# ZhenlongYuan/DVP-MVS

Measured on AMD Instinct MI355X. Metric: Mpixels/sec/PatchMatch-iteration, higher is better.
Workload: dtype f32

## Files before the change

__graft_entry__.py:

```python
import importlib
import os
import subprocess
import sys

ROOT = os.path.dirname(os.path.abspath(__file__))
if ROOT not in sys.path:
    sys.path.insert(0, ROOT)


def build() -> None:
    subprocess.check_call(["make", "-s", "-C", os.path.join(ROOT, "dvp-mvs_amd", "csrc")])
    host = os.path.join(ROOT, "dvp-mvs_amd", "host")
    if os.path.exists(os.path.join(host, "Makefile")):
        subprocess.check_call(["make", "-s", "-C", host])
    subprocess.check_call(["make", "-s", "-C", os.path.join(ROOT, "oracle")])
    subprocess.check_call(["make", "-s", "-C", os.path.join(ROOT, "tests", "emul")])
    subprocess.check_call(["make", "-s", "-C", os.path.join(ROOT, "tests", "sweep_host")])
    subprocess.check_call(["make", "-s", "-C", os.path.join(ROOT, "tests", "host")])
    subprocess.check_call(["make", "-s", "-C", os.path.join(ROOT, "tests", "half16")])
    subprocess.check_call(["make", "-s", "-C", os.path.join(ROOT, "tests", "jpeg_host")])
    subprocess.check_call(["make", "-s", "-C", os.path.join(ROOT, "tests", "edges_host")])
    subprocess.check_call(["make", "-s", "-C", os.path.join(ROOT, "tests", "viewclean_host")])
    subprocess.check_call(["make", "-s", "-C", os.path.join(ROOT, "tests", "labels_host")])
    subprocess.check_call(["make", "-s", "-C", os.path.join(ROOT, "tests", "pyramid_host")])
    subprocess.check_call(["make", "-s", "-C", os.path.join(ROOT, "tests", "prior_host")])
    subprocess.check_call(["make", "-s", "-C", os.path.join(ROOT, "tests", "reuse_host")])
    subprocess.check_call(["make", "-s", "-C", os.path.join(ROOT, "tests", "devmem_host")])
    subprocess.check_call(["make", "-s", "-C", os.path.join(ROOT, "tests", "jpeg_dec_host")])
    subprocess.check_call(["make", "-s", "-C", os.path.join(ROOT, "tests", "convert_host")])
    subprocess.check_call(["make", "-s", "-C", os.path.join(ROOT, "tests", "undistort_host")])
    pkg = importlib.import_module("dvp-mvs_amd")
    lib = pkg.get_capi().lib()
    missing = [s for s in pkg.get_capi().EXPORTS + pkg.get_capi().EXPORTS_WITH_DIGITS if not hasattr(lib, s)]
    if missing:
        raise RuntimeError("libdvp_mvs_hip.so lacks symbols: %s" % missing)


def smoke() -> None:
    import numpy as np
    pkg = importlib.import_module("dvp-mvs_amd")
    synth, capi = pkg.synth, pkg.get_capi()
    from oracle import oracle as O
    W, H, S = 96, 64, 3
    sc = synth.make_scene(W, H, S)
    p = synth.default_params(S + 1, max_iterations=1, state=synth.FIRST_INIT, use_APD=0)
    p["depth_min"] = np.float32(2.5) * np.float32(0.6)
    p["depth_max"] = np.float32(6.5) * np.float32(1.2)
    state = dict(planes=np.zeros((H * W, 4), np.float32), edge=sc["edge"], label=sc["label"],
                 radius=np.full(H * W, 5, np.int32))
    g = capi.from_scene(sc, p, device=0)
    g.upload_state(**state)
    g.run_patchmatch()
    o = O.from_scene(sc, p)
    o.upload_state(**state)
    o.run_patchmatch()
    pg, po = g.get("planes"), o.get("planes")
    same = (pg.view(np.uint32) == po.view(np.uint32)) | (np.isnan(pg) & np.isnan(po))
    if not same.all():
        raise AssertionError("smoke: HIP planes differ from the oracle in %d values" % int((~same).sum()))
    for n in ("selected_views", "weak_info", "radius"):
        if not (g.get(n) == o.get(n)).all():
            raise AssertionError("smoke: %s differs from the oracle" % n)
    print("smoke ok: %dx%d S=%d bit-exact vs oracle; total %.2f ms" % (W, H, S, g.timings()["total_ms"]))


if __name__ == "__main__":
    build()
    if os.path.exists("/dev/kfd"):
        smoke()
```

dvp-mvs_amd/csrc/dvp_engine.hip:

```cpp
#include "dvp_kernels.hpp"
#include "dvp_ctx.hpp"
#ifdef DVP_PROBE
#include "dvp_probe.inc"
#endif
#include "dvp_pyramid_run.h"
#include <cstring>
#include <thread>
#include <chrono>
#include <algorithm>
#include <cmath>

extern "C" {

int dvp_ctx_create(int device, int width, int height, int num_images, dvp_ctx** out) {
	if (!out) return 1;
	*out = nullptr;
	if (width <= 0 || height <= 0 || num_images < 2 || num_images > DVP_MAX_IMAGES || width > 32767 || height > 32767) {
		g_create_error = "dvp_ctx_create: bad dimensions (2 <= num_images <= 32, sizes <= 32767: short2 pixel coordinates)";
		return 1;
	}
	{
		const unsigned long long pitch = ((unsigned long long)width + 2 * kImgPad + 63) / 64 * 64;
		if (pitch * ((unsigned long long)height + 2 * kImgPad) * 8ull >= (1ull << 32)) {
			g_create_error = "dvp_ctx_create: image too large (a padded row-pair plane must stay below 4 GiB)";
// ... 477 lines not shown
	if (anchor_table_off(c) || c->anchor_tab_valid) return 0;
	const int wc = c->d.weak_black + c->d.weak_red;
	if (grow_anchor_table(c, (size_t)wc)) return 1;
	if (anchor_table_off(c)) return 0;
	c->anchor_tab_valid = true;
	sync_dev_struct(c);
	ListArgs la;
	la.base = 0; la.count = wc; la.iter = 0; la.covered_rows = covered_rows;
	const long long n = (long long)wc * (c->NI - 1) * kAnchors;
	if (n > 0) {
		hipLaunchKernelGGL(dvp_weak_anchor_table, dim3((unsigned)((n + 255) / 256)), dim3(256), 0, c->stream, c->d, la);
		HIP_TRY(c, hipGetLastError());
	}
	return 0;
}

static int grow_weak_phase_buffers(dvp_ctx* c, size_t wc) {
	if (!c->sw.weak_phased || !c->weak_phase_fits || wc <= c->weak_phase_alloc) return 0;
	HIP_TRY(c, hipStreamSynchronize(c->stream));
	dfree(c, &c->weak_rec); dfree(c, &c->weak_ctab); dfree(c, &c->weak_ev);
	c->weak_phase_alloc = 0;
	const size_t cap = std::min<size_t>(c->L, wc + wc / 2), S = (size_t)c->NI - 1;
	if (alloc_group_or_fall_back(c, { areq(&c->weak_rec, cap * sizeof(WeakRec)), areq(&c->weak_ctab, cap * kTaps * kTaps * sizeof(f2)), areq(&c->weak_ev, cap * 8 * S * sizeof(float)) },
			"DVP_TEST_WEAK_PHASE_ALLOC_FAIL", &c->weak_phase_fits, "dvp: no room for the phased weak update's hand-over buffers (%.2f GB); using the one-wave kernel\n", (double)cap * (sizeof(WeakRec) + 288 + 32 * S) / 1e9))
		c->weak_phase_alloc = cap;
	return 0;
}

static void ensure_strong_reuse_buffers(dvp_ctx* c) {
	if (c->reuse_costs || !c->sw.strong_reuse || !c->reuse_fits || strong_form(c->sw, c->NI - 1, c->split_fits, false, 0).kernel != STRONG_SPLIT) return;
	const size_t L = c->L, vec = (size_t)kSlotCount * (c->NI - 1) * L * sizeof(float) + 64 ;
	const size_t Lh = (size_t)((c->W + 1) / 2) * c->H;
	alloc_group_or_fall_back(c, { areq(&c->reuse_costs, vec), areq(&c->reuse_keys, L * kSlotCount * sizeof(PlaneKey)), areq(&c->reuse_hdr, L * sizeof(ReuseHdr), true),
			c->strong_rec ? AllocReq{} : areq(&c->strong_rec, (size_t)SR_FIELDS * Lh * sizeof(*c->strong_rec)) },
		"DVP_TEST_REUSE_ALLOC_FAIL", &c->reuse_fits, "dvp: no room for the strong update's plane cache (%.1f GB); every visit evaluates all its planes\n", (double)(vec + L * (kSlotCount * sizeof(PlaneKey) + sizeof(ReuseHdr))) / 1e9);
}
static void ensure_strong_split_buffers(dvp_ctx* c) {
	if (c->slot_costs || strong_form(c->sw, c->NI - 1, c->split_fits, false, 0).kernel != STRONG_SPLIT) return;
	if (!getenv("DVP_TEST_SPLIT_ALLOC_FAIL")) {
		ensure_strong_reuse_buffers(c);
		if (c->reuse_costs) return;
	}
	const size_t Lh = (size_t)((c->W + 1) / 2) * c->H;
	alloc_group_or_fall_back(c, { areq(&c->slot_costs, (size_t)kSlotCount * (c->NI - 1) * Lh * sizeof(*c->slot_costs) + 64 ),
			areq(&c->strong_rec, (size_t)SR_FIELDS * Lh * sizeof(*c->strong_rec)) },
		"DVP_TEST_SPLIT_ALLOC_FAIL", &c->split_fits, "dvp: no room for the split strong update's cost buffer (%.1f GB); using the monolithic kernel\n", (double)kSlotCount * (c->NI - 1) * Lh * 4 / 1e9);
}
static void ensure_sweep_buffers(dvp_ctx* c) {
	if (c->sweep_cost || !c->sw.sweep_split || !c->sweep_fits) return;
	const size_t L = c->L;
	c->sweep_band_rows = sweep_band_rows(c->sw, c->W, c->H, c->NI - 1);
	const size_t band_px = c->sweep_band_rows > 0 ? (size_t)c->sweep_band_rows * c->W : L;
	alloc_group_or_fall_back(c, { areq(&c->sweep_rec, 2 * L * sizeof(f4)), areq(&c->sweep_pc, 61 * L * sizeof(float)), areq(&c->sweep_cost, sweep_cost_floats(band_px, c->NI - 1) * sizeof(float)) },
		"DVP_TEST_SWEEP_ALLOC_FAIL", &c->sweep_fits, "dvp: no room for the view-compacted DepthToWeak's cost buffer (%.1f GB); using the fused kernel\n", (double)(c->NI - 1) * kSweepFields * L * 4 / 1e9);
}


#define DVP_PICK(NAME, SUF) (c->d.sampler ? NAME##_exact##SUF : NAME##SUF)
#define DVP_PICK_FMT(NAME, TAIL) (fmt == 1 ? DVP_PICK(NAME, _u8##TAIL) : (fmt == 2 ? DVP_PICK(NAME, _f16##TAIL) : DVP_PICK(NAME, TAIL)))

static LaunchArgs make_args(const LaunchGeom& g, int colour, int iter) {
	LaunchArgs a;
	a.tiles_x = g.tiles_x; a.tiles = g.tiles; a.rows = g.rows; a.half = g.half ? 1 : 0;
	a.colour = colour; a.iter = iter;
	return a;
}

static void launch_gen_candidates(dvp_ctx* c, hipStream_t stream, const Dev& d, unsigned blocks, const LaunchArgs& a, const unsigned* list = nullptr, const unsigned* n_list = nullptr) {
	const bool all = gen_candidates_all_views(d);
	const dim3 grid(blocks, all ? (unsigned)((c->NI - 1 + kCandGroup - 1) / kCandGroup) : (unsigned)(c->NI - 1)), block(256);
	if (list) hipLaunchKernelGGL(all ? dvp_gen_candidates_views_list : dvp_gen_candidates_list, grid, block, 0, stream, d, list, n_list);
	else hipLaunchKernelGGL(all ? dvp_gen_candidates_views : dvp_gen_candidates, grid, block, 0, stream, d, a);
}

static int launch_strong_prep(dvp_ctx* c, const LaunchGeom& g, const LaunchArgs& a) {
	EventPair prep;
	prep.stage = DVP_ST_STRONG_PREP;
	HIP_TRY(c, hipEventCreate(&prep.a));
	HIP_TRY(c, hipEventCreate(&prep.b));
	HIP_TRY(c, hipEventRecord(prep.a, c->stream));
	HIP_TRY(c, hipMemcpyAsync(c->planes_snap, c->planes, c->L * 16, hipMemcpyDeviceToDevice, c->stream));
	HIP_TRY(c, hipMemcpyAsync(c->costs_snap, c->costs, c->L * 4, hipMemcpyDeviceToDevice, c->stream));
	ensure_strong_split_buffers(c);
	hipLaunchKernelGGL(dvp_strong_search, dim3(g.grid()), dim3(256), 0, c->stream, c->d, a);
	if (strong_form(c->sw, c->NI - 1, c->split_fits, c->d.reuse_hdr != nullptr, 0).plan) hipLaunchKernelGGL(dvp_strong_plan, dim3(g.grid()), dim3(256), 0, c->stream, c->d, a);
	HIP_TRY(c, hipGetLastError());
	HIP_TRY(c, hipEventRecord(prep.b, c->stream));
	c->events.push_back(prep);
	return 0;
}

static int launch_strong_update(dvp_ctx* c, const LaunchGeom& g, const LaunchArgs& a) {
	const dim3 grid(g.grid()), block(256);
	const dim3 wave_grid((unsigned)((g.grid() + 7) / 8 * 32)), wave_block(64);
	ensure_strong_split_buffers(c);
	const StrongForm f = strong_form(c->sw, c->NI - 1, c->split_fits, c->d.reuse_hdr != nullptr, (unsigned long long)c->pitch * (c->H + 2 * kImgPad) * 8 * c->NI);
	switch (f.kernel) {
	case STRONG_SPLIT:
		if (f.eval_items) hipLaunchKernelGGL(DVP_PICK(dvp_strong_eval_items, ), wave_grid, wave_block, 0, c->stream, c->d, a);
		else hipLaunchKernelGGL(DVP_PICK(dvp_strong_eval, ), wave_grid, wave_block, 0, c->stream, c->d, a);
		hipLaunchKernelGGL(f.decide == 4 ? dvp_strong_decide_v4 : f.decide == 6 ? dvp_strong_decide_v6 : f.decide == 8 ? dvp_strong_decide_v8 : f.decide == 10 ? dvp_strong_decide_v10 :
		                   f.decide == 12 ? dvp_strong_decide_v12 : f.decide == 16 ? dvp_strong_decide_v16 : dvp_strong_decide_wide, grid, block, 0, c->stream, c->d, a);
		if (f.refine_lanes) hipLaunchKernelGGL(DVP_PICK(dvp_strong_refine_lanes, ), wave_grid, wave_block, 0, c->stream, c->d, a);
		else hipLaunchKernelGGL(DVP_PICK(dvp_strong_refine, ), wave_grid, wave_block, 0, c->stream, c->d, a);
		break;
	case STRONG_MONO_V8: hipLaunchKernelGGL(DVP_PICK(dvp_strong_update_v8, ), grid, block, 0, c->stream, c->d, a); break;
	case STRONG_MONO_V16: hipLaunchKernelGGL(DVP_PICK(dvp_strong_update_v16, ), grid, block, 0, c->stream, c->d, a); break;
	case STRONG_MONO: hipLaunchKernelGGL(DVP_PICK(dvp_strong_update, ), grid, block, 0, c->stream, c->d, a); break;
	}
	HIP_TRY(c, hipGetLastError());
	return 0;
}

static int launch_weak_update(dvp_ctx* c, ListArgs la) {
	if (ensure_anchor_table(c, la.covered_rows)) return 1;
	if (c->d.anchor_tab && grow_weak_phase_buffers(c, (size_t)(c->d.weak_black + c->d.weak_red))) return 1;
	const WeakForm f = weak_form(c->sw, c->d.anchor_tab != nullptr, c->weak_phase_fits, la.count);
	const int fmt = dvp_image_format(c);
	const dim3 lg((la.count + 255) / 256), block(256), w64(64), lg64((la.count + 63) / 64);
	switch (f.kernel) {
	case WEAK_PHASED:
#define DVP_GROUP_LAUNCH(NAME, PHASE) { la.group = f.group[PHASE]; la.run = f.run[PHASE]; hipLaunchKernelGGL(DVP_PICK_FMT(NAME, ), dim3((la.count + la.group - 1) / la.group), w64, 0, c->stream, c->d, la); }
		DVP_GROUP_LAUNCH(dvp_weak_eval_candidates, 0)
		hipLaunchKernelGGL(dvp_weak_select_views, lg, block, 0, c->stream, c->d, la);
		DVP_GROUP_LAUNCH(dvp_weak_eval_planes, 1)
		hipLaunchKernelGGL(dvp_weak_make_hypotheses, lg, block, 0, c->stream, c->d, la);
		DVP_GROUP_LAUNCH(dvp_weak_eval_first_view, 2)
		DVP_GROUP_LAUNCH(dvp_weak_eval_survivors, 3)
#undef DVP_GROUP_LAUNCH
		hipLaunchKernelGGL(dvp_weak_adopt, lg, block, 0, c->stream, c->d, la);
		hipLaunchKernelGGL(DVP_PICK(dvp_weak_final_cost, ), lg64, w64, 0, c->stream, c->d, la);
		break;
	case WEAK_WAVE: hipLaunchKernelGGL(DVP_PICK_FMT(dvp_weak_update_wave, ), dim3(la.count), w64, 0, c->stream, c->d, la); break;
	case WEAK_WAVE_NOTAB: hipLaunchKernelGGL(DVP_PICK_FMT(dvp_weak_update_wave, _notab), dim3(la.count), w64, 0, c->stream, c->d, la); break;
	}
	return 0;
}

static int launch_list_site(dvp_ctx* c, int stage, int iter, int colour) {
	const dim3 block(256);
	const size_t words = edge_bits_words(c->W, c->H);
	const dim3 wgrid((unsigned)((words + 255) / 256));
	if (stage == DVP_ST_FIND_NEAREST_STRONG && c->d.weak_black + c->d.weak_red > 0) {
		hipLaunchKernelGGL(dvp_pack_edge_bits, wgrid, block, 0, c->stream, c->weak_info, c->strong_bits, c->W, c->H, edge_tiles_x(c->W), words, (int)DVP_STRONG);
		hipLaunchKernelGGL(dvp_pack_bits_transposed, wgrid, block, 0, c->stream, c->weak_info, c->strong_bits_t, c->W, c->H, edge_tiles_x(c->W), words, (int)DVP_STRONG);
		HIP_TRY(c, hipGetLastError());
	}
	if (stage == DVP_ST_GEN_NEIGHBOURS || stage == DVP_ST_RANSAC_FIT) {
		hipLaunchKernelGGL(dvp_pack_edge_bits, wgrid, block, 0, c->stream, c->edge, c->edge_bits, c->W, c->H, edge_tiles_x(c->W), words, -1);
		HIP_TRY(c, hipGetLastError());
		const int cells = c->d.sat_cells_x * c->d.sat_cells_y;
		hipLaunchKernelGGL(dvp_edge_cell_counts, dim3((cells + 255) / 256), dim3(256), 0, c->stream, c->d);
		hipLaunchKernelGGL(dvp_edge_sat_rows, dim3((c->d.sat_cells_y + 1 + 63) / 64), dim3(64), 0, c->stream, c->d);
		hipLaunchKernelGGL(dvp_edge_sat_cols, dim3((c->d.sat_cells_x + 1 + 63) / 64), dim3(64), 0, c->stream, c->d);
		HIP_TRY(c, hipGetLastError());
		if (stage == DVP_ST_GEN_NEIGHBOURS) {
			hipLaunchKernelGGL(dvp_pack_edge_bits, wgrid, block, 0, c->stream, c->weak_info, c->strong_bits, c->W, c->H, edge_tiles_x(c->W), words, (int)DVP_STRONG);
			HIP_TRY(c, hipGetLastError());
		}
	}
	if (stage == DVP_ST_FIND_NEAREST_STRONG) HIP_TRY(c, hipMemsetAsync(c->weak_nearest_strong, 0xFF, c->L * sizeof(s2), c->stream));
	if (stage == DVP_ST_RANSAC_FIT) HIP_TRY(c, hipMemcpyAsync(c->fit_planes, c->planes, c->L * 16, hipMemcpyDeviceToDevice, c->stream));
	ListArgs la;
	la.iter = iter;
	la.covered_rows = 2 * make_geom(c->W, c->H, true).rows;
	la.base = (stage == DVP_ST_WEAK_UPDATE && colour == 1) ? c->d.weak_black : 0;
	la.count = (stage == DVP_ST_WEAK_UPDATE) ? (colour == 0 ? c->d.weak_black : (colour == 1 ? c->d.weak_red : c->d.weak_black + c->d.weak_red)) : c->d.weak_black + c->d.weak_red;
	if (la.count <= 0) return 0;
// ... 595 lines not shown
```

dvp-mvs_amd/csrc/dvp_kernels.hpp:

```cpp
#ifndef DVP_KERNELS_HPP_
#define DVP_KERNELS_HPP_

#include "dvp_stages.hpp"
#include <hip/hip_runtime.h>

using namespace dvp;

struct LaunchArgs {
	int tiles_x, tiles, rows, half, colour, iter;
};

template <int STAGE, int SMP, int MV = 32>
__device__ __forceinline__ void stage_body(const Dev& d, const LaunchArgs& a) {
	const int lane = threadIdx.x & 63;
	const int wave = threadIdx.x >> 6;
	int px, py;
	unsigned long long n = 0;
	__shared__ f2 lds_tab[stage_uses_tab(STAGE) ? kTaps * kTaps * 256 : 1];
	const PatchTab tab{&lds_tab[stage_uses_tab(STAGE) ? threadIdx.x : 0], 256};
	if (block_to_pixel(blockIdx.x, lane, wave, a.tiles_x, a.tiles, a.rows, a.half, a.colour, d.width, d.height, &px, &py))
		run_pixel<STAGE, SMP, MV>(d, px, py, a.iter, d.eval_counter ? &n : nullptr, tab);
	if (d.eval_counter && n) atomicAdd(d.eval_counter, n);
}

// ... 509 lines not shown
}

extern "C" __global__ void __launch_bounds__(256) dvp_gen_candidates_views(const Dev d, const LaunchArgs a) {
	int px, py;
	if (block_to_pixel(blockIdx.x, threadIdx.x & 63, threadIdx.x >> 6, a.tiles_x, a.tiles, a.rows, 0, 0, d.width, d.height, &px, &py))
		gen_candidates_views_px<kCandGroup>(d, px, py, (int)blockIdx.y * kCandGroup);
}
extern "C" __global__ void __launch_bounds__(256) dvp_gen_candidates_views_list(const Dev d, const unsigned* list, const unsigned* n_list) {
	const unsigned t = blockIdx.x * 256 + threadIdx.x;
	if (t >= *n_list) return;
	const int center = (int)list[t];
	const int py = center / d.width, px = center - py * d.width;
	gen_candidates_views_px<kCandGroup>(d, px, py, (int)blockIdx.y * kCandGroup);
}

extern "C" __global__ void __launch_bounds__(256) dvp_anchor_mask(const Dev d, const ListArgs a, uint8_t* mask) {
	const int t = blockIdx.x * 256 + threadIdx.x;
	if (t >= a.count) return;
	const int center = d.weak_list[a.base + t];
	const s2* nb = d.neighbours + (size_t)d.neighbours_map[center] * DVP_NEIGHBOUR_NUM;
	for (int k = 1; k < DVP_NEIGHBOUR_NUM; ++k) {
		const s2 q = nb[k];
		if (q.x >= 0 && q.y >= 0 && q.x < d.width && q.y < d.height) mask[(size_t)q.y * d.width + q.x] = 1;
	}
}
extern "C" __global__ void __launch_bounds__(256) dvp_mask_compact(const uint8_t* mask, size_t L, unsigned* list, unsigned* n_list) {
	const size_t p = (size_t)blockIdx.x * 256 + threadIdx.x;
	const bool go = p < L && mask[p] != 0;
	const unsigned long long m = __ballot(go);
	if (!m) return;
	const int lane = threadIdx.x & 63;
	unsigned base = 0;
	if (lane == __builtin_ctzll(m)) base = atomicAdd(n_list, (unsigned)__popcll(m));
	base = __shfl(base, __builtin_ctzll(m), 64);
	if (go) list[base + __popcll(m & ((1ull << lane) - 1ull))] = (unsigned)p;
}
extern "C" __global__ void __launch_bounds__(256) dvp_gen_candidates_list(const Dev d, const unsigned* list, const unsigned* n_list) {
	const unsigned t = blockIdx.x * 256 + threadIdx.x;
	if (t >= *n_list) return;
	const int center = (int)list[t];
	const int py = center / d.width, px = center - py * d.width;
	gen_candidates_px(d, px, py, (int)blockIdx.y);
}

extern "C" __global__ void dvp_pack_bits_transposed(const uint8_t* __restrict__ map, uint32_t* __restrict__ bits, int W, int H, int tiles_x, size_t words, int equals) {
	const size_t w = (size_t)blockIdx.x * blockDim.x + threadIdx.x;
	if (w < words) bits[w] = pack_edge_word_t(map, W, H, tiles_x, w, equals);
}

extern "C" __global__ void dvp_edge_cell_counts(const Dev d) {
	const int c = blockIdx.x * blockDim.x + threadIdx.x;
	if (c >= d.sat_cells_x * d.sat_cells_y) return;
	const int cy = c / d.sat_cells_x, cx = c - cy * d.sat_cells_x;
	int n = 0;
	for (int r = 0; r < 8; ++r) {
		const int y = cy * 8 + r;
		if (y >= d.height) break;
		const unsigned w = d.edge_bits[(size_t)(((y >> 5) * d.edge_tiles_x + (cx >> 2)) * 32 + (y & 31))];
		n += __popc((w >> ((cx & 3) * 8)) & 255u);
	}
	d.edge_sat[(cy + 1) * (d.sat_cells_x + 1) + cx + 1] = n;
}
extern "C" __global__ void dvp_edge_sat_rows(const Dev d) {
	const int r = blockIdx.x * blockDim.x + threadIdx.x;
	if (r > d.sat_cells_y) return;
	int* row = d.edge_sat + (size_t)r * (d.sat_cells_x + 1);
	int acc = 0;
	for (int x = 0; x <= d.sat_cells_x; ++x) { acc += (r == 0 || x == 0) ? 0 : row[x]; row[x] = acc; }
}
extern "C" __global__ void dvp_edge_sat_cols(const Dev d) {
	const int x = blockIdx.x * blockDim.x + threadIdx.x;
	if (x > d.sat_cells_x) return;
	const int P = d.sat_cells_x + 1;
	int acc = 0;
	for (int r = 0; r <= d.sat_cells_y; ++r) { acc += d.edge_sat[(size_t)r * P + x]; d.edge_sat[(size_t)r * P + x] = acc; }
}

extern "C" __global__ void __launch_bounds__(256) dvp_strong_search(const Dev d, const LaunchArgs a) {
	int px, py;
	if (block_to_pixel(blockIdx.x, threadIdx.x & 63, threadIdx.x >> 6, a.tiles_x, a.tiles, a.rows, a.half, a.colour, d.width, d.height, &px, &py))
		strong_search_px(d, px, py);
}

extern "C" __global__ void __launch_bounds__(256) dvp_strong_plan(const Dev d, const LaunchArgs a) {
	int px, py;
	if (block_to_pixel(blockIdx.x, threadIdx.x & 63, threadIdx.x >> 6, a.tiles_x, a.tiles, a.rows, a.half, a.colour, d.width, d.height, &px, &py) &&
	    d.weak_info[px + py * d.width] != DVP_WEAK)
		strong_plan_px(d, px, py);
}

extern "C" __global__ void __launch_bounds__(256) dvp_edge_rays(const Dev d, int what) {
	edge_ray_line(d, blockIdx.y, blockIdx.x * blockDim.x + threadIdx.x, what);
}

constexpr int kWeakTile = 16, kWeakSuper = 64, kWeakChunk = 1024;
DVP_HD void weak_slot_origin(int slot, int supers_x, int* tx, int* ty) {
	const int super = slot >> 4, t = slot & 15;
	*tx = (super % supers_x) * kWeakSuper + (t & 3) * kWeakTile;
	*ty = (super / supers_x) * kWeakSuper + (t >> 2) * kWeakTile;
}
extern "C" __global__ void __launch_bounds__(256) dvp_weak_counts(const uint8_t* __restrict__ weak, int W, int H, int supers_x, int n_slots, int n_chunks, int* __restrict__ counts) {
	const int lane = threadIdx.x & 63;
	const int unit = blockIdx.x * 4 + (threadIdx.x >> 6);
	if (unit < n_slots) {
		int tx, ty;
		weak_slot_origin(unit, supers_x, &tx, &ty);
		int nb = 0, nr = 0;
		for (int step = 0; step < 4; ++step) {
			const int x = tx + (lane & 15), y = ty + step * 4 + (lane >> 4);
			const bool wk = x < W && y < H && weak[(size_t)y * W + x] == DVP_WEAK;
			nb += __popcll(__ballot(wk && !((x + y) & 1)));
			nr += __popcll(__ballot(wk && ((x + y) & 1)));
		}
		if (lane == 0) { counts[unit] = nb; counts[n_slots + unit] = nr; }
	} else if (unit < n_slots + n_chunks) {
		const int chunk = unit - n_slots;
		const size_t L = (size_t)W * H;
		int n = 0;
		for (int step = 0; step < kWeakChunk / 64; ++step) {
			const size_t i = (size_t)chunk * kWeakChunk + step * 64 + lane;
			n += __popcll(__ballot(i < L && weak[i] == DVP_WEAK));
		}
		if (lane == 0) counts[2 * n_slots + chunk] = n;
	}
}
extern "C" __global__ void __launch_bounds__(1024) dvp_scan3(int* __restrict__ data, int s0, int s1, int s2, int s3, int* __restrict__ totals) {
	__shared__ int part[1024];
	__shared__ int carry;
	const int starts[4] = { s0, s1, s2, s3 };
	const int lo = starts[blockIdx.x], hi = starts[blockIdx.x + 1];
	if (threadIdx.x == 0) carry = 0;
	__syncthreads();
	for (int base = lo; base < hi; base += 1024) {
		const int i = base + (int)threadIdx.x;
		const int v = i < hi ? data[i] : 0;
		part[threadIdx.x] = v;
		__syncthreads();
		for (int off = 1; off < 1024; off <<= 1) {
			const int add = threadIdx.x >= (unsigned)off ? part[threadIdx.x - off] : 0;
			__syncthreads();
			part[threadIdx.x] += add;
			__syncthreads();
		}
		if (i < hi) data[i] = carry + part[threadIdx.x] - v;
		__syncthreads();
		if (threadIdx.x == 1023) carry += part[1023];
		__syncthreads();
	}
	if (threadIdx.x == 0) totals[blockIdx.x] = carry;
}
extern "C" __global__ void __launch_bounds__(256) dvp_weak_fill(const uint8_t* __restrict__ weak, int W, int H, int supers_x, int n_slots, int n_chunks,
                                                               const int* __restrict__ offs, const int* __restrict__ totals, int* __restrict__ list, int* __restrict__ map) {
	const int lane = threadIdx.x & 63;
	const int unit = blockIdx.x * 4 + (threadIdx.x >> 6);
	const unsigned long long below = (1ull << lane) - 1ull;
	if (unit < n_slots) {
		int tx, ty;
		weak_slot_origin(unit, supers_x, &tx, &ty);
		int ob = offs[unit], orr = totals[0] + offs[n_slots + unit];
		for (int step = 0; step < 4; ++step) {
			const int x = tx + (lane & 15), y = ty + step * 4 + (lane >> 4);
			const bool wk = x < W && y < H && weak[(size_t)y * W + x] == DVP_WEAK;
			const bool red = (x + y) & 1;
			const unsigned long long mb = __ballot(wk && !red), mr = __ballot(wk && red);
			if (wk) list[red ? orr + __popcll(mr & below) : ob + __popcll(mb & below)] = y * W + x;
			ob += __popcll(mb);
			orr += __popcll(mr);
		}
	} else if (unit < n_slots + n_chunks) {
		const int chunk = unit - n_slots;
		const size_t L = (size_t)W * H;
// ... 81 lines not shown
```

dvp-mvs_amd/csrc/dvp_strong.hpp:

```cpp
#ifndef DVP_STRONG_HPP_
#define DVP_STRONG_HPP_

#include "dvp_ncc.hpp"

namespace dvp {

DVP_HD void sort_small(float* v, int n) {
	for (int i = 1; i < n; i++) {
		const float tmp = v[i];
		int j = i;
		for (; j >= 1 && tmp < v[j - 1]; j--) v[j] = v[j - 1];
		v[j] = tmp;
	}
}

DVP_HD f4 random_normal_yzl_sel(const Dev& d, int px, int py, Rng& rng, float depth, uint32_t sel) {
	const int W = d.width, H = d.height;
	const DvpCamera rc = load_camera(d, 0);
	f3 vd[20];
	{
		const f4 v0 = view_direction(rc, px, py, depth);
		vd[0] = mk3(v0.x, v0.y, v0.z);
	}
	int index = 1;
// ... 223 lines not shown
		for (int j = 0; j < 8; j++) {
			const float cst = cost_array[j * MV + i];
			if (cst < thr) { tmpw += dvp_expf(cst * cst / (-0.18f)); count++; }
			if (cst > 1.2f) count_false++;
		}
		float pr = 0.0f;
		if (count > 2 && count_false < 3) pr = tmpw / count;
		else if (count_false < 3) pr = dvp_expf(thr * thr / (-0.32f));
		probs[i] = pr * priors[i];
	}
	float psum = 0.0f;
	for (int i = 0; i < S; ++i) psum += probs[i];
	const float inv = 1.0f / psum;
	float cum = 0.0f;
	for (int i = 0; i < S; ++i) { cum += probs[i] * inv; probs[i] = cum; }
	Rng rv(d.seed, (uint32_t)center, rng_site(phase, iter, SUB_VIEW));
	for (int s = 0; s < 15; ++s) {
		const float rp = rv.uniform() - FLT_EPSILON;
		for (int v = 0; v < S; ++v)
			if (probs[v] > rp) { vw[v] += 1; break; }
	}
	uint32_t m = 0;
	float wn = 0;
	for (int i = 0; i < S; ++i)
		if (vw[i] > 0) { set_bit(&m, i); wn += vw[i]; }
	*sel_mask = m;
	*weight_norm = wn;
}

DVP_HD int strong_sample_search(const Dev& d, int px, int py, int k, int pass) {
	const int W = d.width, H = d.height;
	const int center = py * W + px;
	const int dxs[8] = { 0, 0, -1, 1, -1, 1, -1, 1 };
	const int dys[8] = { -1, 1, 0, 0, -1, 1, 1, -1 };
	const int dx = dxs[k], dy = dys[k];
	int step_num = 11, step_len = 2;
	if (pass == 0) {
		const float max_edge_dist = DVP_MAX(H, W) / 30.0f;
		const s2 ep = d.edge_neigh[(size_t)center * 8 + k];
		const double ex = (double)(ep.x - px), ey = (double)(ep.y - py);
		float dist = (float)sqrt(ex * ex + ey * ey);
		if (k >= 4) dist = (float)((double)dist / sqrt(2.0));
		if (d.edge[center]) {
			dist = 22.0f;
		} else if (ep.y == -1 || dist >= max_edge_dist) {
			dist = max_edge_dist;
			if (k >= 4) dist = (float)((double)dist / sqrt(2.0));
		}
		step_num = DVP_MIN(DVP_MAX(11, (int)(1.0f * dist / 2)), 22);
		step_len = DVP_MAX((int)(1.0f * dist / step_num), 2);
		if (k < 4 && step_len % 2 == 1) step_len -= 1;
	}
	int fx = 0, fy = 0;
	if (k > 4) { if (k % 2) fx = dx; else fy = dy; }
	int best = -1;
	float min_cost = FLT_MAX;
	float cs[22];
	int pcs[22];
#pragma unroll
	for (int step = 0; step < 22; ++step) {
		const int tx = px + 5 * dx + step * step_len * dx + fx;
		const int ty = py + 5 * dy + step * step_len * dy + fy;
		const bool ok = step < step_num && tx >= 0 && ty >= 0 && tx < W && ty < H;
		pcs[step] = ok ? tx + ty * W : -1;
		cs[step] = ok ? d.costs_snap[tx + ty * W] : 0.0f;
	}
#pragma unroll
	for (int step = 0; step < 22; ++step) {
		if (pcs[step] >= 0 && min_cost > cs[step]) { best = pcs[step]; min_cost = cs[step]; }
	}
	return (min_cost < FLT_MAX) ? best : -1;
}

DVP_HD void strong_search_px(const Dev& d, int px, int py) {
	const int center = py * d.width + px;
	if (d.weak_info[center] == DVP_WEAK) return;
	const size_t L = (size_t)d.width * d.height;
	const bool is_edge = d.edge[center] != 0;
	for (int slot = 0; slot < 16; ++slot) {
		int pos = -1;
		if (slot < 8) pos = strong_sample_search(d, px, py, slot, 0);
		else if (!is_edge) pos = strong_sample_search(d, px, py, slot - 8, 1);
		d.search_pos[(size_t)slot * L + center] = pos;
	}
}

template <int SMP, int MV = 32>
DVP_HD void strong_update_px(const Dev& d, int px, int py, PatchTab tab, int iter, unsigned long long* nevals) {
	const int W = d.width;
	const int center = py * W + px;
	const DvpParams& P = d.params;
	const DvpCamera rc = load_camera(d, 0);
	const int S = P.num_images - 1;
	const uint32_t all_views = (S >= 32) ? 0xFFFFFFFFu : ((1u << S) - 1u);

	PatchCtx c;
	{
		int radius, inc;
		patch_geometry(d, center, &radius, &inc);
		build_patch_ctx(d, px, py, radius, inc, 0, tab, &c);
	}
	float cost_array[8 * MV];
	for (int i = 0; i < 8 * MV; ++i) cost_array[i] = 0.0f;
	cost_array[0] = 2.0f;
	uint32_t flag = 0;
	int positions[8];
	for (int k = 0; k < 8; ++k) positions[k] = 0;
	const bool is_edge = d.edge[center] != 0;
	const float good_thr = 0.8f * dvp_expf((iter) * (iter) / (-90.0f));

	uint8_t vw[MV];
	for (int i = 0; i < MV; ++i) vw[i] = 0;
	uint32_t sel_mask = 0;
	float weight_norm = 0.0f;
	float final_costs[8];
	int min_cost_idx = 0;
	float cost_now = 0.0f, costs_center = 0.0f, depth_now = 0.0f;
	f4 plane_now = mk4(0, 0, 0, 0);
	bool selected_views_written = false;
	float ref_depths[6];
	f4 ref_normals[6];

	float cv[MV];
	for (int slot = 0; slot < 23; ++slot) {
		if (slot == 21) continue;
		f4 plane = mk4(0, 0, 1, 1);
		uint32_t mask = 0;
		int pos = -1;
		if (slot < 16) {
			pos = d.search_pos[(size_t)slot * ((size_t)W * d.height) + center];
			if (pos >= 0) { plane = d.planes_snap[pos]; mask = all_views; }
		} else if (slot == 16) {
			float priors[MV];
			for (int i = 0; i < MV; ++i) priors[i] = 0.0f;
			const int nb[4] = { center - W, center + W, center - 1, center + 1 };
			for (int i = 0; i < 4; ++i) {
				if ((flag >> (2 * i)) & 1) {
					const uint32_t sv = d.selected_views[nb[i]];
					for (int j = 0; j < S; ++j) priors[j] += is_set(sv, j) ? 0.9f : 0.1f;
				}
			}
			joint_view_selection<MV>(d, center, iter, PH_STRONG, cost_array, priors, vw, &sel_mask, &weight_norm);
			uint8_t* gvw = d.view_weight + (size_t)center * 32;
			for (int i = 0; i < 32; ++i) gvw[i] = i < MV ? vw[i < MV ? i : 0] : (uint8_t)0;
			for (int k = 0; k < 8; ++k) {
				float fc = 0.0f;
				for (int j = 0; j < S; ++j)
					if (vw[j] > 0) fc += vw[j] * cost_array[k * MV + j];
				final_costs[k] = fc / weight_norm;
			}
			min_cost_idx = 0;
			{
				float mc = final_costs[0];
				for (int k = 1; k < 8; ++k)
					if (final_costs[k] <= mc) { mc = final_costs[k]; min_cost_idx = k; }
			}
			plane = d.planes_snap[center];
			mask = sel_mask;
		} else {
			const int i = slot - 17;
			plane = ref_normals[i];
			plane.w = distance_to_origin(rc, px, py, ref_depths[i], plane);
			mask = sel_mask;
		}

		if (mask) {
// ... 62 lines not shown
			ref_depths[2] = depth_rand; ref_normals[2] = n_rand;
			ref_depths[3] = depth_now;  ref_normals[3] = n_pert;
			ref_depths[4] = depth_now;  ref_normals[4] = n_pert;
			ref_depths[5] = depth_pert; ref_normals[5] = plane_now;
		} else {
			float tc = 0.0f;
			for (int j = 0; j < S; ++j)
				if (vw[j] > 0) tc += vw[j] * cv[j];
			tc /= weight_norm;
			const float db = depth_from_plane(rc, plane, px, py);
			if (db >= P.depth_min && db <= P.depth_max && tc < cost_now) {
				depth_now = db;
				plane_now = plane;
				cost_now = tc;
			}
		}
	}

	if (P.state == DVP_REFINE_INIT) {
		if (cost_now < costs_center - 0.1) {
			costs_center = cost_now;
			d.planes[center] = plane_now;
		}
	} else {
		costs_center = cost_now;
		d.planes[center] = plane_now;
	}
	d.costs[center] = costs_center;
}

constexpr int kSlotCur = 16;
constexpr int kSlotCount = 17;
enum { SR_PLANE = 0, SR_DEPTH = 4, SR_COST = 5, SR_CENTER = 6, SR_DRAND = 7, SR_DPERT = 8, SR_NRAND = 9, SR_DUP = 12 , SR_FIELDS = 15 };
DVP_HD size_t half_index(const Dev& d, int px, int py) { return (size_t)py * d.half_w + (size_t)(px >> 1); }
#ifndef DVP_SLOT_LAYOUT
#define DVP_SLOT_LAYOUT 1
#endif
DVP_HD int slot_place(int slot) {
#if DVP_SLOT_LAYOUT
	return slot < 8 ? 2 * slot : (slot < 16 ? 2 * (slot - 8) + 1 : slot);
#else
	return slot;
#endif
}
DVP_HD size_t slot_cost_index(const Dev& d, int slot, int v, int px, int py) {
	const size_t Lh = (size_t)d.half_w * (size_t)d.height;
	const int S = d.params.num_images - 1;
#if DVP_SLOT_LAYOUT
	return (half_index(d, px, py) * kSlotCount + (size_t)slot_place(slot)) * (size_t)S + (size_t)v;
#else
	return (size_t)(slot * S + v) * Lh + half_index(d, px, py);
#endif
}
struct SlotCostView { const float* base; size_t slot_stride, view_stride; };
DVP_HD SlotCostView slot_cost_view(const Dev& d, int px, int py) {
	const size_t Lh = (size_t)d.half_w * (size_t)d.height;
	const int S = d.params.num_images - 1;
	SlotCostView r;
#if DVP_SLOT_LAYOUT
	r.base = d.slot_costs + half_index(d, px, py) * kSlotCount * (size_t)S;
	r.slot_stride = (size_t)S;
	r.view_stride = 1;
#else
	r.base = d.slot_costs + half_index(d, px, py);
	r.slot_stride = (size_t)S * Lh;
	r.view_stride = Lh;
#endif
	return r;
}
DVP_HD bool same_plane_bits(const f4 a, const f4 b) {
	return f32_bits(a.x) == f32_bits(b.x) && f32_bits(a.y) == f32_bits(b.y) && f32_bits(a.z) == f32_bits(b.z) && f32_bits(a.w) == f32_bits(b.w);
}
DVP_HD uint32_t strong_slot_planes(const Dev& d, int center, f4 pl[kSlotCount]) {
	const size_t L = (size_t)d.width * d.height;
	uint32_t have = 0;
#pragma unroll
	for (int slot = 0; slot < kSlotCount; ++slot) {
		const int pos = slot < 16 ? d.search_pos[(size_t)slot * L + center] : center;
		pl[slot] = mk4(0.0f, 0.0f, 0.0f, 0.0f);
		if (pos >= 0) { pl[slot] = d.planes_snap[pos]; have |= 1u << slot; }
	}
	return have;
}
DVP_HD uint32_t strong_slot_sources_of(const f4 pl[kSlotCount], uint32_t have, uint32_t w[3]) {
	uint32_t uniq = 0;
	w[0] = w[1] = w[2] = 0;
#pragma unroll
	for (int slot = 0; slot < kSlotCount; ++slot) {
		int src = slot;
#pragma unroll
		for (int u = slot - 1; u >= 0; --u)
			if (((have >> u) & 1u) && same_plane_bits(pl[u], pl[slot])) src = u;
		if (!((have >> slot) & 1u)) continue;
		if (src == slot) uniq |= 1u << slot;
		if (slot < 8) w[0] |= (uint32_t)src << (4 * slot);
		else if (slot < 16) w[1] |= (uint32_t)src << (4 * (slot - 8));
		else w[2] = (uint32_t)src;
	}
	return uniq;
}
DVP_HD uint32_t strong_slot_sources(const Dev& d, int center, uint32_t w[3]) {
	f4 pl[kSlotCount];
	const uint32_t have = strong_slot_planes(d, center, pl);
	return strong_slot_sources_of(pl, have, w);
}
DVP_HD int strong_slot_source(uint32_t w0, uint32_t w1, uint32_t w2, int slot) {
	return slot < 8 ? (int)((w0 >> (4 * slot)) & 15u) : slot < 16 ? (int)((w1 >> (4 * (slot - 8))) & 15u) : (int)w2;
}
constexpr uint32_t kPlaceMask = (1u << kSlotCount) - 1u;
DVP_HD int strong_slot_place_of(uint32_t w0, uint32_t w1, uint32_t w2, int slot) {
	return slot < 6 ? (int)((w0 >> (5 * slot)) & 31u) : slot < 12 ? (int)((w1 >> (5 * (slot - 6))) & 31u) : (int)((w2 >> (5 * (slot - 12))) & 31u);
}
DVP_HD void strong_source_places(const uint32_t src[3], uint32_t place_w[3]) {
	place_w[0] = place_w[1] = place_w[2] = 0;
#pragma unroll
	for (int s = 0; s < kSlotCount; ++s)
		place_w[s / 6] |= (uint32_t)slot_place(strong_slot_source(src[0], src[1], src[2], s)) << (5 * (s % 6));
}
DVP_HD PlaneKey plane_key(const f4 p) {
	PlaneKey k;
	k.w[0] = f32_bits(p.x); k.w[1] = f32_bits(p.y); k.w[2] = f32_bits(p.z); k.w[3] = f32_bits(p.w);
	return k;
}
DVP_HD uint32_t strong_reuse_plan(const f4 pl[kSlotCount], uint32_t uniq, const uint32_t src[3], PlaneKey* keys, ReuseHdr* hdr,
                                  uint32_t epoch, int radius, uint32_t place_w[3]) {
	const ReuseHdr h = *hdr;
	const uint32_t valid = (h.epoch == epoch && h.radius == (uint32_t)radius) ? (h.valid & kPlaceMask) : 0u;
	int place[kSlotCount];
#pragma unroll
	for (int s = 0; s < kSlotCount; ++s) place[s] = -1;
	uint32_t held = 0;
	if (valid) {
#pragma unroll
		for (int p = 0; p < kSlotCount; ++p) {
			if (!((valid >> p) & 1u)) continue;
			const PlaneKey k = keys[p];
#pragma unroll
			for (int s = 0; s < kSlotCount; ++s) {
				if (!((uniq >> s) & 1u) || place[s] >= 0) continue;
				if (k.w[0] == f32_bits(pl[s].x) && k.w[1] == f32_bits(pl[s].y) && k.w[2] == f32_bits(pl[s].z) && k.w[3] == f32_bits(pl[s].w)) { place[s] = p; held |= 1u << p; }
			}
		}
	}
	uint32_t free_places = kPlaceMask & ~held, eval = 0;
#pragma unroll
	for (int s = 0; s < kSlotCount; ++s) {
		if (!((uniq >> s) & 1u) || place[s] >= 0) continue;
		const int p = dvp_ctz(free_places);
		free_places &= free_places - 1;
		place[s] = p;
		eval |= 1u << s;
		keys[p] = plane_key(pl[s]);
	}
	place_w[0] = place_w[1] = place_w[2] = 0;
#pragma unroll
	for (int s = 0; s < kSlotCount; ++s) {
		const int from = strong_slot_source(src[0], src[1], src[2], s);
		int p = 0;
#pragma unroll
		for (int u = 0; u <= s; ++u)
			if (u == from && place[u] >= 0) p = place[u];
		place_w[s / 6] |= (uint32_t)p << (5 * (s % 6));
	}
	ReuseHdr o;
	o.valid = kPlaceMask & ~free_places; o.radius = (uint32_t)radius; o.epoch = epoch; o.eval = eval;
	*hdr = o;
	return eval;
}
DVP_HD void strong_plan_px(const Dev& d, int px, int py) {
	const int center = py * d.width + px;
	f4 pl[kSlotCount];
	const uint32_t have = strong_slot_planes(d, center, pl);
	uint32_t src[3], pw[3];
	const uint32_t uniq = strong_slot_sources_of(pl, have, src);
	strong_reuse_plan(pl, uniq, src, d.reuse_keys + (size_t)center * kSlotCount, d.reuse_hdr + center, d.reuse_epoch, d.radius[center], pw);
	const size_t Lh = (size_t)d.half_w * (size_t)d.height;
	uint32_t* dup = reinterpret_cast<uint32_t*>(d.strong_rec) + half_index(d, px, py);
	dup[SR_DUP * Lh] = pw[0]; dup[(SR_DUP + 1) * Lh] = pw[1]; dup[(SR_DUP + 2) * Lh] = pw[2];
}
template <int SMP>
DVP_HD void strong_eval_item(const Dev& d, const PatchCtx& c, int px, int py, int slot, bool store, unsigned long long* nevals) {
	const int W = d.width;
	const int center = py * W + px;
	const int S = d.params.num_images - 1;
	const size_t L = (size_t)W * d.height;
	const int pos = slot < 16 ? d.search_pos[(size_t)slot * L + center] : center;
	const f4 plane = d.planes_snap[pos];
	const bool reuse = d.reuse_costs != nullptr;
	float* const buf = reuse ? d.reuse_costs : d.slot_costs;
	int at = slot_place(slot);
	if (reuse) {
		const size_t Lh = (size_t)d.half_w * (size_t)d.height;
		const int word = (slot >= 6) + (slot >= 12);
		const uint32_t pw = reinterpret_cast<const uint32_t*>(d.strong_rec)[(size_t)(SR_DUP + word) * Lh + half_index(d, px, py)];
		at = (int)((pw >> (5 * (slot - 6 * word))) & 31u);
	}
	for (int v = 0; v < S; ++v) {
		const float cost = ncc_old<SMP>(d, c, px, py, v + 1, plane);
#if DVP_SLOT_LAYOUT
		const size_t rec = reuse ? (size_t)center : half_index(d, px, py);
		if (store) DVP_NT_STORE(4, &buf[(rec * kSlotCount + (size_t)at) * (size_t)S + (size_t)v], cost);
#else
		if (store) DVP_NT_STORE(4, &buf[reuse ? ((size_t)center * kSlotCount + (size_t)at) * (size_t)S + (size_t)v : slot_cost_index(d, slot, v, px, py)], cost);
#endif
	}
	if (nevals && store) *nevals += (unsigned long long)S;
}
template <int SMP>
DVP_HD void strong_eval_px(const Dev& d, int px, int py, PatchTab tab, unsigned long long* nevals) {
	const int W = d.width;
	const int center = py * W + px;
	PatchCtx c;
	{
		int radius, inc;
		patch_geometry(d, center, &radius, &inc);
		build_patch_ctx(d, px, py, radius, inc, 0, tab, &c);
	}
	uint32_t uniq;
	if (d.reuse_hdr) uniq = d.reuse_hdr[center].eval;
	else {
		uint32_t src[3], w[3];
		uniq = strong_slot_sources(d, center, src);
		strong_source_places(src, w);
		const size_t Lh = (size_t)d.half_w * (size_t)d.height, hi = half_index(d, px, py);
		uint32_t* dup = reinterpret_cast<uint32_t*>(d.strong_rec) + hi;
		dup[SR_DUP * Lh] = w[0]; dup[(SR_DUP + 1) * Lh] = w[1]; dup[(SR_DUP + 2) * Lh] = w[2];
	}
	for (uint32_t m = uniq; m; m &= m - 1) strong_eval_item<SMP>(d, c, px, py, dvp_ctz(m), true, nevals);
}

template <int MV>
DVP_HD void load_slot_costs(const float* sc, size_t view_stride, int S, float* out) {
#if defined(__HIP_DEVICE_COMPILE__) && DVP_SLOT_LAYOUT
	typedef float f4v __attribute__((ext_vector_type(4), aligned(4)));
	constexpr int Q = (MV + 3) / 4;
	f4v q[Q];
#pragma unroll
	for (int i = 0; i < Q; ++i) q[i] = DVP_NT_LOAD(8, &reinterpret_cast<const f4v*>(sc)[i]);
#pragma unroll
	for (int v = 0; v < MV; ++v) out[v] = v < S ? q[v >> 2][v & 3] : 0.0f;
#else
#pragma unroll
	for (int v = 0; v < MV; ++v) out[v] = v < S ? sc[(size_t)v * view_stride] : 0.0f;
#endif
}

DVP_HD void strong_decide_wide_px(const Dev& d, int px, int py, int iter);
template <int MV>
DVP_HD void strong_decide_px(const Dev& d, int px, int py, int iter) {
#if !defined(__HIP_DEVICE_COMPILE__)
	if (d.params.num_images - 1 > MV) { strong_decide_wide_px(d, px, py, iter); return; }
#endif
	const int W = d.width;
	const int center = py * W + px;
	const DvpParams& P = d.params;
	const DvpCamera rc = load_camera(d, 0);
	const int S = P.num_images - 1;
	const bool reuse = d.reuse_costs != nullptr;
	SlotCostView cv;
	if (reuse) { cv.base = d.reuse_costs + (size_t)center * kSlotCount * (size_t)S; cv.slot_stride = (size_t)S; cv.view_stride = 1; }
	else cv = slot_cost_view(d, px, py);
// ... 540 lines not shown
```

Baseline: 61.74.

## Fuse strong search and reuse planning into one kernel with leaner dedup

Adds a fused dvp_strong_search_plan kernel that runs the strong sample search and the reuse plan per pixel, keeping search positions in registers instead of re-reading search_pos. The plane dedup and key matching are rewritten to compare 64-bit packed plane bits and to load the reuse header once before the search. Both plan kernels also get occupancy launch bounds. The aim is to remove one launch and a global round trip for search positions. In exchange, register pressure rises from the shifting 16-entry position array and the unrolled pairwise comparisons.

Measured after the change: 62.05 (median of 6 runs). About the same (+0.5%).

```diff
diff --git a/__graft_entry__.py b/__graft_entry__.py
--- a/__graft_entry__.py
+++ b/__graft_entry__.py
@@ -25,6 +25,7 @@
     subprocess.check_call(["make", "-s", "-C", os.path.join(ROOT, "tests", "pyramid_host")])
     subprocess.check_call(["make", "-s", "-C", os.path.join(ROOT, "tests", "prior_host")])
     subprocess.check_call(["make", "-s", "-C", os.path.join(ROOT, "tests", "reuse_host")])
+    subprocess.check_call(["make", "-s", "-C", os.path.join(ROOT, "tests", "plan_host")])
     subprocess.check_call(["make", "-s", "-C", os.path.join(ROOT, "tests", "devmem_host")])
     subprocess.check_call(["make", "-s", "-C", os.path.join(ROOT, "tests", "jpeg_dec_host")])
     subprocess.check_call(["make", "-s", "-C", os.path.join(ROOT, "tests", "convert_host")])
diff --git a/dvp-mvs_amd/csrc/dvp_engine.hip b/dvp-mvs_amd/csrc/dvp_engine.hip
--- a/dvp-mvs_amd/csrc/dvp_engine.hip
+++ b/dvp-mvs_amd/csrc/dvp_engine.hip
@@ -583,8 +583,12 @@
 	HIP_TRY(c, hipMemcpyAsync(c->planes_snap, c->planes, c->L * 16, hipMemcpyDeviceToDevice, c->stream));
 	HIP_TRY(c, hipMemcpyAsync(c->costs_snap, c->costs, c->L * 4, hipMemcpyDeviceToDevice, c->stream));
 	ensure_strong_split_buffers(c);
-	hipLaunchKernelGGL(dvp_strong_search, dim3(g.grid()), dim3(256), 0, c->stream, c->d, a);
-	if (strong_form(c->sw, c->NI - 1, c->split_fits, c->d.reuse_hdr != nullptr, 0).plan) hipLaunchKernelGGL(dvp_strong_plan, dim3(g.grid()), dim3(256), 0, c->stream, c->d, a);
+	const bool plan = strong_form(c->sw, c->NI - 1, c->split_fits, c->d.reuse_hdr != nullptr, 0).plan;
+	if (plan && DVP_PLAN_FUSED) hipLaunchKernelGGL(dvp_strong_search_plan, dim3(g.grid()), dim3(256), 0, c->stream, c->d, a);
+	else {
+		hipLaunchKernelGGL(dvp_strong_search, dim3(g.grid()), dim3(256), 0, c->stream, c->d, a);
+		if (plan) hipLaunchKernelGGL(dvp_strong_plan, dim3(g.grid()), dim3(256), 0, c->stream, c->d, a);
+	}
 	HIP_TRY(c, hipGetLastError());
 	HIP_TRY(c, hipEventRecord(prep.b, c->stream));
 	c->events.push_back(prep);
diff --git a/dvp-mvs_amd/csrc/dvp_kernels.hpp b/dvp-mvs_amd/csrc/dvp_kernels.hpp
--- a/dvp-mvs_amd/csrc/dvp_kernels.hpp
+++ b/dvp-mvs_amd/csrc/dvp_kernels.hpp
@@ -615,11 +615,30 @@
 		strong_search_px(d, px, py);
 }
 
-extern "C" __global__ void __launch_bounds__(256) dvp_strong_plan(const Dev d, const LaunchArgs a) {
+extern "C" __global__ void __launch_bounds__(256, 4) dvp_strong_plan(const Dev d, const LaunchArgs a) {
 	int px, py;
 	if (block_to_pixel(blockIdx.x, threadIdx.x & 63, threadIdx.x >> 6, a.tiles_x, a.tiles, a.rows, a.half, a.colour, d.width, d.height, &px, &py) &&
-	    d.weak_info[px + py * d.width] != DVP_WEAK)
+	    d.weak_info[px + py * d.width] != DVP_WEAK) {
+#if DVP_PLAN_LEAN
+		strong_plan_lean_px(d, px, py);
+#else
 		strong_plan_px(d, px, py);
+#endif
+	}
+}
+
+#ifndef DVP_PLAN_FUSED
+#define DVP_PLAN_FUSED DVP_PLAN_LEAN
+#endif
+extern "C" __global__ void __launch_bounds__(256, 4) dvp_strong_search_plan(const Dev d, const LaunchArgs a) {
+	int px, py;
+	if (!block_to_pixel(blockIdx.x, threadIdx.x & 63, threadIdx.x >> 6, a.tiles_x, a.tiles, a.rows, a.half, a.colour, d.width, d.height, &px, &py)) return;
+	const int center = px + py * d.width;
+	if (d.weak_info[center] == DVP_WEAK) return;
+	const ReuseHdr h = d.reuse_hdr[center];
+	int pos[16];
+	strong_search_keep_px(d, px, py, pos);
+	strong_plan_lean_px(d, px, py, pos, h);
 }
 
 extern "C" __global__ void __launch_bounds__(256) dvp_edge_rays(const Dev d, int what) {
diff --git a/dvp-mvs_amd/csrc/dvp_strong.hpp b/dvp-mvs_amd/csrc/dvp_strong.hpp
--- a/dvp-mvs_amd/csrc/dvp_strong.hpp
+++ b/dvp-mvs_amd/csrc/dvp_strong.hpp
@@ -329,6 +329,24 @@
 		if (slot < 8) pos = strong_sample_search(d, px, py, slot, 0);
 		else if (!is_edge) pos = strong_sample_search(d, px, py, slot - 8, 1);
 		d.search_pos[(size_t)slot * L + center] = pos;
+	}
+}
+
+DVP_HD void strong_search_keep_px(const Dev& d, int px, int py, int pos[16]) {
+	const int center = py * d.width + px;
+	const size_t L = (size_t)d.width * d.height;
+	const bool is_edge = d.edge[center] != 0;
+#pragma unroll
+	for (int i = 0; i < 16; ++i) pos[i] = -1;
+#pragma unroll 1
+	for (int slot = 0; slot < 16; ++slot) {
+		int p = -1;
+		if (slot < 8) p = strong_sample_search(d, px, py, slot, 0);
+		else if (!is_edge) p = strong_sample_search(d, px, py, slot - 8, 1);
+		d.search_pos[(size_t)slot * L + center] = p;
+#pragma unroll
+		for (int i = 0; i < 15; ++i) pos[i] = pos[i + 1];
+		pos[15] = p;
 	}
 }
 
@@ -557,6 +575,10 @@
 	}
 	return have;
 }
+#ifndef DVP_PLAN_LEAN
+#define DVP_PLAN_LEAN 1
+#endif
+DVP_HD uint32_t strong_slot_sources_lean(const f4 pl[kSlotCount], uint32_t have, uint32_t w[3]);
 DVP_HD uint32_t strong_slot_sources_of(const f4 pl[kSlotCount], uint32_t have, uint32_t w[3]) {
 	uint32_t uniq = 0;
 	w[0] = w[1] = w[2] = 0;
@@ -577,7 +599,11 @@
 DVP_HD uint32_t strong_slot_sources(const Dev& d, int center, uint32_t w[3]) {
 	f4 pl[kSlotCount];
 	const uint32_t have = strong_slot_planes(d, center, pl);
+#if defined(__HIP_DEVICE_COMPILE__) && DVP_PLAN_LEAN
+	return strong_slot_sources_lean(pl, have, w);
+#else
 	return strong_slot_sources_of(pl, have, w);
+#endif
 }
 DVP_HD int strong_slot_source(uint32_t w0, uint32_t w1, uint32_t w2, int slot) {
 	return slot < 8 ? (int)((w0 >> (4 * slot)) & 15u) : slot < 16 ? (int)((w1 >> (4 * (slot - 8))) & 15u) : (int)w2;
@@ -652,6 +678,122 @@
 	const size_t Lh = (size_t)d.half_w * (size_t)d.height;
 	uint32_t* dup = reinterpret_cast<uint32_t*>(d.strong_rec) + half_index(d, px, py);
 	dup[SR_DUP * Lh] = pw[0]; dup[(SR_DUP + 1) * Lh] = pw[1]; dup[(SR_DUP + 2) * Lh] = pw[2];
+}
+struct PlaneBits { uint64_t lo, hi; };
+DVP_HD PlaneBits plane_bits(uint32_t x, uint32_t y, uint32_t z, uint32_t w) {
+	PlaneBits r;
+	r.lo = (uint64_t)x | ((uint64_t)y << 32); r.hi = (uint64_t)z | ((uint64_t)w << 32);
+	return r;
+}
+DVP_HD bool same_plane_bits(const PlaneBits& a, const PlaneBits& b) { return (a.lo == b.lo) & (a.hi == b.hi); }
+DVP_HD uint32_t strong_slot_sources_lean(const f4 pl[kSlotCount], uint32_t have, uint32_t w[3]) {
+	PlaneBits b[kSlotCount];
+	int src[kSlotCount];
+#pragma unroll
+	for (int s = 0; s < kSlotCount; ++s) { b[s] = plane_bits(f32_bits(pl[s].x), f32_bits(pl[s].y), f32_bits(pl[s].z), f32_bits(pl[s].w)); src[s] = s; }
+#pragma unroll
+	for (int u = kSlotCount - 2; u >= 0; --u) {
+		const bool hu = (have >> u) & 1u;
+#pragma unroll
+		for (int s = u + 1; s < kSlotCount; ++s)
+			if (hu & same_plane_bits(b[u], b[s])) src[s] = u;
+	}
+	uint32_t uniq = 0;
+	w[0] = w[1] = w[2] = 0;
+#pragma unroll
+	for (int s = 0; s < kSlotCount; ++s) {
+		if (!((have >> s) & 1u)) continue;
+		if (src[s] == s) uniq |= 1u << s;
+		if (s < 8) w[0] |= (uint32_t)src[s] << (4 * s);
+		else if (s < 16) w[1] |= (uint32_t)src[s] << (4 * (s - 8));
+		else w[2] = (uint32_t)src[s];
+	}
+	return uniq;
+}
+DVP_HD uint32_t strong_plan_lean(const f4 pl[kSlotCount], uint32_t have, const ReuseHdr h, PlaneKey* keys, ReuseHdr* hdr, uint32_t epoch,
+                                 int radius, uint32_t src_w[3], uint32_t place_w[3], uint32_t* uniq_out) {
+	const uint32_t valid = (h.epoch == epoch && h.radius == (uint32_t)radius) ? (h.valid & kPlaceMask) : 0u;
+	PlaneBits b[kSlotCount];
+	int place[kSlotCount];
+#pragma unroll
+	for (int s = 0; s < kSlotCount; ++s) { b[s] = plane_bits(f32_bits(pl[s].x), f32_bits(pl[s].y), f32_bits(pl[s].z), f32_bits(pl[s].w)); place[s] = -1; }
+	if (valid) {
+		PlaneKey next = keys[kSlotCount - 1];
+#pragma unroll 1
+		for (int p = kSlotCount - 1; p >= 0; --p) {
+			const PlaneKey k = next;
+			if (p > 0) next = keys[p - 1];
+			if (!((valid >> p) & 1u)) continue;
+			const PlaneBits kb = plane_bits(k.w[0], k.w[1], k.w[2], k.w[3]);
+#pragma unroll
+			for (int s = 0; s < kSlotCount; ++s)
+				if (same_plane_bits(kb, b[s])) place[s] = p;
+		}
+	}
+	uint32_t held = 0;
+#pragma unroll
+	for (int s = 0; s < kSlotCount; ++s)
+		if (((have >> s) & 1u) && place[s] >= 0) held |= 1u << place[s];
+	uint32_t free_places = kPlaceMask & ~held, eval = 0, uniq = 0;
+	src_w[0] = src_w[1] = src_w[2] = 0;
+	place_w[0] = place_w[1] = place_w[2] = 0;
+#pragma unroll
+	for (int s = 0; s < kSlotCount; ++s) {
+		int src = s, from_place = 0;
+#pragma unroll
+		for (int u = s - 1; u >= 0; --u)
+			if (((have >> u) & 1u) & same_plane_bits(b[u], b[s])) { src = u; from_place = place[u]; }
+		int p;
+		if (!((have >> s) & 1u)) {
+			src = 0;
+			p = (s > 0 && (have & 1u)) ? place[0] : 0;
+		} else if (src != s) p = from_place;
+		else {
+			uniq |= 1u << s;
+			p = place[s];
+			if (p < 0) {
+				p = dvp_ctz(free_places);
+				free_places &= free_places - 1;
+				eval |= 1u << s;
+				keys[p] = plane_key(pl[s]);
+			}
+		}
+		place[s] = p;
+		if (s < 8) src_w[0] |= (uint32_t)src << (4 * s);
+		else if (s < 16) src_w[1] |= (uint32_t)src << (4 * (s - 8));
+		else src_w[2] = (uint32_t)src;
+		place_w[s / 6] |= (uint32_t)p << (5 * (s % 6));
+	}
+	ReuseHdr o;
+	o.valid = kPlaceMask & ~free_places; o.radius = (uint32_t)radius; o.epoch = epoch; o.eval = eval;
+	*hdr = o;
+	*uniq_out = uniq;
+	return eval;
+}
+DVP_HD void strong_plan_lean_px(const Dev& d, int px, int py, const int pos[kSlotCur], const ReuseHdr h) {
+	const int center = py * d.width + px;
+	f4 pl[kSlotCount];
+	uint32_t have = 0;
+#pragma unroll
+	for (int slot = 0; slot < kSlotCount; ++slot) {
+		const int at = slot < kSlotCur ? pos[slot] : center;
+		pl[slot] = mk4(0.0f, 0.0f, 0.0f, 0.0f);
+		if (at >= 0) { pl[slot] = d.planes_snap[at]; have |= 1u << slot; }
+	}
+	uint32_t src[3], pw[3], uniq;
+	strong_plan_lean(pl, have, h, d.reuse_keys + (size_t)center * kSlotCount, d.reuse_hdr + center, d.reuse_epoch, d.radius[center], src, pw, &uniq);
+	const size_t Lh = (size_t)d.half_w * (size_t)d.height;
+	uint32_t* dup = reinterpret_cast<uint32_t*>(d.strong_rec) + half_index(d, px, py);
+	dup[SR_DUP * Lh] = pw[0]; dup[(SR_DUP + 1) * Lh] = pw[1]; dup[(SR_DUP + 2) * Lh] = pw[2];
+}
+DVP_HD void strong_plan_lean_px(const Dev& d, int px, int py) {
+	const int center = py * d.width + px;
+	const size_t L = (size_t)d.width * d.height;
+	const ReuseHdr h = d.reuse_hdr[center];
+	int pos[kSlotCur];
+#pragma unroll
+	for (int slot = 0; slot < kSlotCur; ++slot) pos[slot] = d.search_pos[(size_t)slot * L + center];
+	strong_plan_lean_px(d, px, py, pos, h);
 }
 template <int SMP>
 DVP_HD void strong_eval_item(const Dev& d, const PatchCtx& c, int px, int py, int slot, bool store, unsigned long long* nevals) {
```
